# matinmoezzi/MyCobotGym

Measured on AMD Instinct MI355X. Metric: env-steps/sec (whole node), MyCobot Reach, N_envs=8192/GPU, higher is better.
Workload: dtype f64

## Files before the change

mycobotgym_amd/csrc/mcg_dynamics.hpp:

```cpp
#pragma once
#ifndef MCG_DUP
#define MCG_DUP 0
#endif

#include <type_traits>
#include <hip/hip_runtime.h>
#include "mcg.h"

namespace mcg {

typedef double real;

constexpr int NB = 12;
constexpr int AXK[NB] = {2, 0, 0, 0, 2, 0, 1, 1, 1, 1, 1, 1};
constexpr int AXS[NB] = {-1, -1, 1, -1, -1, -1, 1, -1, -1, 1, 1, 1};
constexpr int PAR[NB] = {-1, 0, 1, 2, 3, 4, 5, 6, 5, 8, 5, 5};
constexpr real MINVAL = 1e-15, MINIMP = 1e-4, MAXIMP = 0.9999;

#define MCG_DEV __device__ __forceinline__

enum { ST_LOAD = 0, ST_CTRL, ST_TRIG, ST_RNE, ST_ACT, ST_CRB, ST_ROWS, ST_G0, ST_NEWTON, ST_EULER, ST_COLLIDE, ST_CUBE,
       ST_COUPLED, ST_CUBE_FIN, ST_POST, ST_N_BUILD, ST_N_FACTOR, ST_N_SOLVE, ST_N_CHECK, ST_E_RHS, ST_R_AX5, ST_R_CONNECT, ST_R_LIMITS, ST_C_MASK, ST_C_ASSEMBLE, ST_C_SCHUR, ST_C_SOLVE, ST_C_CHECK, ST_C_LS, ST_W2_WAIT1, ST_W2_COLLIDE, ST_W2_CUBE, ST_W2_WAIT2, ST_W1_WAIT, ST_A_ENTRY, ST_A_G, ST_A_TWIST, ST_A_LOOP, ST_A_MAP, ST_A_STORE,
       ST_CO_SETUP, ST_CO_ROWS, ST_CO_H0, ST_CO_RESID, ST_CO_ASM, ST_CO_FACTOR, ST_CO_SOLVE, ST_CO_CHECK, ST_CO_LS, ST_CO_OUT, ST_CO_IDLE,
       ST_X_S1C, ST_X_NUMBERS, ST_X_S2, ST_S_S1B, ST_S_MESH, ST_S_S1C, ST_S_NUMBERS,
       ST_M_S3, ST_H_S1, ST_H_CRB, ST_H_S2, ST_H_FACTOR, ST_H_S3, ST_Q_S1, ST_Q_BIAS, ST_Q_S2, ST_Q_COLS, ST_Q_S3, ST_COUNT,
       CN_SUBSTEP = 0, CN_NEWTON_IT, CN_LINESEARCH, CN_CUBE_IT, CN_CUBE_LS, CN_COUPLED, CN_COUPLED_IT, CN_COUPLED_LS, CN_CONTACTS, CN_COOP_ROWS, CN_COOP_LSEVAL, CN_COOP_LONG, CN_COOP_CAP, CN_COOP_12, CN_G_FAILED, CN_G_LIM, CN_G_STAT, CN_G_CUBE, CN_G_MISSING, CN_G_EXTRA, CN_G_EQ1, CN_G_EQ2, CN_G_EQ2N1, CN_MP_PAIRS, CN_MP_HITS, CN_MP_FACE, CN_MP_EXIT_B, CN_MP_EXIT_P, CN_MP_EXIT_E, CN_MP_KIND_E, CN_MP_KIND_P, CN_MP_CUBE, CN_COUNT };
#ifdef MCG_STAGE_CLOCKS
__device__ unsigned long long g_stage_clocks[ST_COUNT + CN_COUNT];
__device__ unsigned long long g_tick_last[4096 * 4];
__device__ unsigned long long g_wg_stat[4096 * 4];
#define MCG_TICK_SLOT_ (g_tick_last[(blockIdx.x & 4095) * 4 + (threadIdx.x >> 6)])
#define MCG_TICK_INIT() do { if ((threadIdx.x & 63) == 0) MCG_TICK_SLOT_ = __builtin_readcyclecounter(); } while (0)
#define MCG_TICK(k) do { if ((threadIdx.x & 63) == 0) { const unsigned long long t_ = __builtin_readcyclecounter(); atomicAdd(&g_stage_clocks[k], t_ - MCG_TICK_SLOT_); MCG_TICK_SLOT_ = t_; } } while (0)
#define MCG_TICK2_INIT() MCG_TICK_INIT()
#define MCG_TICK2(k) MCG_TICK(k)
#define MCG_TICK_FLUSH() do {} while (0)
#define MCG_COUNT(k) do { if (threadIdx.x == 0) atomicAdd(&g_stage_clocks[ST_COUNT + (k)], 1ull); } while (0)
#define MCG_COUNTW(k, v) do { if ((threadIdx.x & 63) == 0) atomicAdd(&g_stage_clocks[ST_COUNT + (k)], (unsigned long long)(v)); } while (0)
#define MCG_TICK_PIN(arr, n) do { for (int k_ = 0; k_ < (n); k_++) asm volatile("" : "+v"((arr)[k_])); } while (0)
#else
#define MCG_TICK_INIT() do {} while (0)
#define MCG_TICK(k) do {} while (0)
#define MCG_TICK2_INIT() do {} while (0)
#define MCG_TICK2(k) do {} while (0)
#define MCG_TICK_FLUSH() do {} while (0)
#define MCG_COUNT(k) do {} while (0)
#define MCG_COUNTW(k, v) do {} while (0)
#define MCG_TICK_PIN(arr, n) do {} while (0)
#endif
template <int... Is, class F>
MCG_DEV void static_for_impl(std::integer_sequence<int, Is...>, F&& f) { (f(std::integral_constant<int, Is>{}), ...); }
template <int N, class F>
MCG_DEV void static_for(F&& f) { static_for_impl(std::make_integer_sequence<int, N>{}, f); }

MCG_DEV void cross(const real* a, const real* b, real* r) {
  real x = a[1] * b[2] - a[2] * b[1], y = a[2] * b[0] - a[0] * b[2], z = a[0] * b[1] - a[1] * b[0];
  r[0] = x; r[1] = y; r[2] = z;
}
// ... 261 lines not shown
}
template <int N>
MCG_DEV void chol_solve(const real* L, real* x) {
  static_for<N>([&](auto I) {
    constexpr int i = I;
    real s = x[i];
    static_for<i>([&](auto Kk) { constexpr int k = Kk; s -= L[i * (i + 1) / 2 + k] * x[k]; });
    x[i] = s / L[i * (i + 1) / 2 + i];
  });
  static_for<N>([&](auto I) {
    constexpr int i = N - 1 - I;
    real s = x[i];
    static_for<N - 1 - i>([&](auto Kk) { constexpr int k = i + 1 + Kk; s -= L[k * (k + 1) / 2 + i] * x[k]; });
    x[i] = s / L[i * (i + 1) / 2 + i];
  });
}

struct Robot {
  real q[NB], qd[NB], ctrl[7], warm[NB];
};

constexpr int LDS_M = 0;
constexpr int LDS_HEQ = NB * (NB + 1) / 2;
constexpr int LDS_SLOTS = 2 * (NB * (NB + 1) / 2);
constexpr int LDS_FAC = LDS_SLOTS, LDS_FDINV = LDS_FAC + NB * (NB + 1) / 2, LDS_QB = LDS_FDINV + NB, LDS_QDB = LDS_QB + NB;
constexpr int LDS_FS = LDS_QDB + NB, LDS_WARM = LDS_FS + NB, LDS_QLAG = LDS_WARM + NB, LDS_IKT = LDS_QLAG + 6;
constexpr int LDS_RLIM = LDS_WARM, LDS_RA = LDS_WARM, LDS_RACT = LDS_IKT, LDS_RG0 = LDS_IKT + 8, LDS_SLOTS_SPLIT = LDS_RG0 + NB;
constexpr int RACT_DOF[8] = {0, 1, 2, 3, 4, 5, 6, 8};
static_assert(LDS_RA + NB == LDS_QLAG && LDS_RACT >= LDS_QLAG + 6 && LDS_RACT + 8 <= LDS_RG0,
              "the remote solve's hand-over must stay inside the warm-start and IK-increment slots (the lagged q between them is live)");
static_assert(LDS_SLOTS_SPLIT * 64 * sizeof(real) <= 160 * 1024, "the split Reach kernel's LDS exceeds the 160 KB of a gfx950 workgroup");
constexpr int LDS_SN = LDS_FAC, LDS_CS = LDS_SN + NB;
static_assert(LDS_SN >= LDS_FAC && LDS_CS + NB <= LDS_FDINV + NB && LDS_FDINV + NB == LDS_QB, "the sine / cosine exchange must lie inside the factor slots");
template <class A, class B> MCG_DEV std::common_type_t<A, B> sel(bool c, A a, B b) { return c ? a : b; }
template <class T> MCG_DEV T sel3(int idx, T a, T b, T c) { return idx == 0 ? a : (idx == 1 ? b : c); }

#ifdef MCG_GENERIC_LDS
typedef real* LdsPtr;
#else
typedef __attribute__((address_space(3))) real* LdsPtr;
#endif
template <int STRIDE>
struct LaneScratchT {
  LdsPtr base;
  MCG_DEV explicit LaneScratchT(real* shared_column) : base((LdsPtr)shared_column) {}
  MCG_DEV explicit LaneScratchT(LdsPtr column) : base(column) {}
  MCG_DEV real ld(int k) const { return base[k * STRIDE]; }
  MCG_DEV void st(int k, real v) const { base[k * STRIDE] = v; }
};
typedef LaneScratchT<64> LaneScratch;

struct NoCoupling { static constexpr bool enabled = false, publishes = false; };
struct NoSideWork { MCG_DEV void operator()(const real*, const real*) const {} };

struct NoWeld { static constexpr bool enabled = false; };
struct Weld { static constexpr bool enabled = true; real pos[3], quat[4]; };

MCG_DEV void mulquat(const real* a, const real* b, real* r);
MCG_DEV void normalize4(real* q);
MCG_DEV void quat_to_mat(const real* q, real* m) {
  const real q00 = q[0]*q[0], q01 = q[0]*q[1], q02 = q[0]*q[2], q03 = q[0]*q[3];
  const real q11 = q[1]*q[1], q12 = q[1]*q[2], q13 = q[1]*q[3], q22 = q[2]*q[2], q23 = q[2]*q[3], q33 = q[3]*q[3];
  m[0] = q00 + q11 - q22 - q33; m[4] = q00 - q11 + q22 - q33; m[8] = q00 - q11 - q22 + q33;
  m[1] = 2*(q12 - q03); m[2] = 2*(q13 + q02); m[3] = 2*(q12 + q03);
  m[5] = 2*(q23 - q01); m[6] = 2*(q13 - q02); m[7] = 2*(q23 + q01);
}
// ... 148 lines not shown
        add[3] = It[3] - (m * r[0] * r[1] + r[0] * h3[1] + h3[0] * r[1]);
        add[4] = It[4] - (m * r[0] * r[2] + r[0] * h3[2] + h3[0] * r[2]);
        add[5] = It[5] - (m * r[1] * r[2] + r[1] * h3[2] + h3[1] * r[2]);
        if constexpr (first_child) {
          cm[p] = m;
          for (int k = 0; k < 3; k++) cmc[p][k] = h3[k] + m * r[k];
          for (int k = 0; k < 6; k++) cI[p][k] = add[k];
        } else {
          cm[p] += m;
          for (int k = 0; k < 3; k++) cmc[p][k] += h3[k] + m * r[k];
          for (int k = 0; k < 6; k++) cI[p][k] += add[k];
        }
        pin(cm[p]); pin3(cmc[p]); pin6(cI[p]);
      }
      asm volatile("" ::: "memory");
      MCG_FENCE();
    });
}

template <class LS>
MCG_DEV void euler_accel(ModelPtr Pm, real h, const LS MS, const real* a, real* rhs) {
  real Mh[NB * (NB + 1) / 2], dinv[NB];
  static_for<NB>([&](auto I) { constexpr int i = I;
    static_for<i + 1>([&](auto Jj) { constexpr int j = Jj; if constexpr (PAT_M.nz[i][j]) Mh[tri(i, j)] = MS.ld(LDS_M + tri(i, j)); }); });
  static_for<NB>([&](auto I) { constexpr int i = I; real sacc = 0;
    static_for<NB>([&](auto Jj) { constexpr int j = Jj;
      if constexpr (PAT_M.nz[i > j ? i : j][i > j ? j : i]) sacc = fma(Mh[tri(i, j)], a[j], sacc); }); rhs[i] = sacc; });
  { ModelPtr Q = launder(Pm); static_for<NB>([&](auto I) { constexpr int i = I; Mh[tri(i, i)] = fma(h, Q->body[i].damping, Mh[tri(i, i)]); }); }
  ldl_factor<PAT_M>(Mh, dinv);
  ldl_solve<PAT_M>(Mh, dinv, rhs);
}

struct NoSplit { static constexpr bool enabled = false, rne_remote = false, factor_remote = false, early_heq = false, warm_lds = false, mesh_split = false, solve_remote = false,
                                       trig_once = false;
                 static constexpr int QB = 0, QDB = 0, FS = 0, WARM = 0, QLAG = 0; };
struct SplitMain { static constexpr bool enabled = true, rne_remote = true, factor_remote = true, early_heq = true, warm_lds = true, mesh_split = false, solve_remote = true,
                                         trig_once = true;
                   static constexpr int QB = LDS_QB, QDB = LDS_QDB, FS = LDS_FS, WARM = LDS_WARM, QLAG = LDS_QLAG; };
struct SplitMainLocal : SplitMain { static constexpr bool solve_remote = false; };
struct SplitMainOwnTrig : SplitMain { static constexpr bool trig_once = false; };

template <int FIRST, class LS, class QF>
MCG_DEV void trig_exchange(const LS MS, QF q_of, real* sn, real* cs) {
  {
    const TrigC T = load_trig();
    static_for<4>([&](auto I) { constexpr int i = FIRST + I; real s, c; sincos_cw(T, AXS[i] * q_of(std::integral_constant<int, i>{}), s, c); MS.st(LDS_SN + i, s); MS.st(LDS_CS + i, c); });
  }
  __syncthreads();
  static_for<NB>([&](auto I) { constexpr int i = I; sn[i] = MS.ld(LDS_SN + i); cs[i] = MS.ld(LDS_CS + i); });
}

template <class SPL, class LS>
MCG_DEV void build_H(const LS MS, real* H, const bool* act_, const real* Dl) {
  static_for<NB>([&](auto I) { constexpr int i = I;
    static_for<i + 1>([&](auto Jj) { constexpr int j = Jj;
      if constexpr (PAT_E.nz[i][j]) {
        H[tri(i, j)] = MS.ld(LDS_HEQ + tri(i, j));
        if constexpr (SPL::early_heq && PAT_M.nz[i][j]) H[tri(i, j)] += MS.ld(LDS_M + tri(i, j));
      } else if constexpr (PAT_H.nz[i][j]) H[tri(i, j)] = 0.0; }); });
  static_for<10>([&](auto I) { constexpr int j = I; H[tri(j, j)] += act_[j] ? Dl[j] : 0.0; });
}

template <class SPL, class LS>
MCG_DEV bool no_other_rows(ModelPtr Pm, const LS MS) {
  real jr[10][2];
  { ModelPtr Q = launder(Pm); static_for<10>([&](auto I) { constexpr int j = I; if constexpr (j != 6 && j != 8) { jr[j][0] = Q->jnt_range[j][0]; jr[j][1] = Q->jnt_range[j][1]; } }); }
  bool other = false;
  static_for<10>([&](auto I) { constexpr int j = I;
    if constexpr (j != 6 && j != 8) {
      const real q = MS.ld(SPL::QB + j);
      other = other || (q - jr[j][0] < 0) || (jr[j][1] - q < 0);
    } });
// ... 2 lines not shown

MCG_DEV void limit_pair(bool e0, bool e1, real D0, real D1, real s0, real s1, real rb0, real rb1, real W00, real W01, real W11,
                        real& f0, real& f1) {
  const real A00 = rcp_nr(D0) + W00, A11 = rcp_nr(D1) + W11;
  const real n0 = rb0 * rcp_nr(A00), n1 = rb1 * rcp_nr(A11);
  const real idet = rcp_nr(A00 * A11 - W01 * W01);
  const real b0 = (A11 * rb0 - W01 * rb1) * idet, b1 = (A00 * rb1 - W01 * rb0) * idet;
  const bool cN = (!e0 || rb0 >= 0) && (!e1 || rb1 >= 0);
  const bool cB = e0 && e1 && (b0 < 0) && (b1 < 0);
  const bool c0 = e0 && (n0 < 0) && (!e1 || rb1 - W01 * n0 >= 0);
  const bool c1 = e1 && (n1 < 0) && (rb0 - W01 * n1 >= 0);
  real nu0 = e1 ? b0 : n0, nu1 = e1 ? b1 : 0.0;
  nu0 = c1 ? 0.0 : nu0; nu1 = c1 ? n1 : nu1;
  nu0 = c0 ? n0 : nu0;  nu1 = c0 ? 0.0 : nu1;
  nu0 = cB ? b0 : nu0;  nu1 = cB ? b1 : nu1;
  nu0 = cN ? 0.0 : nu0; nu1 = cN ? 0.0 : nu1;
  f0 = s0 * nu0; f1 = s1 * nu1;
}

MCG_DEV void gear_rows_solve(real* x, const real* z6, const real* z8, real Dl6, real arefl6, real sgl6, real Dl8, real arefl8, real sgl8) {
  const bool v6 = sgl6 != 0, v8 = sgl8 != 0, both = v6 && v8;
  const real D0 = v6 ? Dl6 : (v8 ? Dl8 : 1.0), D1 = both ? Dl8 : 1.0;
  const real ar0 = v6 ? arefl6 : arefl8, ar1 = both ? arefl8 : 0.0;
  const real s0 = v6 ? sgl6 : sgl8, s1 = both ? sgl8 : 0.0;
  const real xa0 = v6 ? x[6] : (v8 ? x[8] : 0.0), xa1 = both ? x[8] : 0.0;
  real W00 = v6 ? z6[6] : (v8 ? z8[8] : 0.0), W01 = both ? z6[8] : 0.0;
  const real W11 = both ? z8[8] : 0.0;
  W01 *= s0 * s1;
  const real rb0 = s0 * xa0 - ar0, rb1 = s1 * xa1 - ar1;
  real f0, f1;
  limit_pair(v6 || v8, both, D0, D1, s0, s1, rb0, rb1, W00, W01, W11, f0, f1);
  const real g6 = v6 ? f0 : 0.0, g8 = v6 ? f1 : f0;
  static_for<NB>([&](auto I) { constexpr int i = I; x[i] = fma(-z8[i], g8, fma(-z6[i], g6, x[i])); });
}

MCG_DEV bool bad_value(real x) { return !(fabs(x) <= 1e10); }

template <class LS, class CPL = NoCoupling, class WLD = NoWeld, class SPL = NoSplit, bool COMMIT = true>
MCG_DEV bool robot_substep(ModelPtr Pm, Robot& S, real* qlag6, const LS MS, CPL* CP = nullptr, const WLD* WD = nullptr,
                           Robot* next = nullptr) {
  MCG_COUNT(CN_SUBSTEP);
  if constexpr (SPL::enabled) __syncthreads();
  const real h = launder(Pm)->timestep;
  real cs[NB], sn[NB];
  if constexpr (SPL::trig_once) trig_exchange<0>(MS, [&](auto I) { return S.q[I]; }, sn, cs);
  else {
    const TrigC T = load_trig();
    static_for<NB>([&](auto I) { constexpr int i = I; sincos_cw(T, AXS[i] * S.q[i], sn[i], cs[i]); });
  }
  if constexpr (!(SPL::warm_lds && !CPL::enabled)) static_for<6>([&](auto I) { constexpr int i = I; qlag6[i] = S.q[i]; });
  static_for<NB>([&](auto I) { constexpr int i = I; pin(sn[i]); pin(cs[i]); });
  MCG_FENCE();

  MCG_TICK(ST_TRIG);
  real fs[NB];
  if constexpr (SPL::rne_remote) { static_for<NB>([&](auto I) { constexpr int i = I; fs[i] = 0; }); }
  else rne_bias(Pm, cs, sn, S.qd, fs);
  MCG_TICK(ST_RNE);
  {
    ModelPtr Q = launder(Pm);
    static_for<6>([&](auto I) {
      constexpr int u = I;
      real c = fmin(fmax(S.ctrl[u], Q->act_ctrlrange[u][0]), Q->act_ctrlrange[u][1]);
      real f = Q->act_gain[u] * c + Q->act_bias[u][0] + Q->act_bias[u][1] * S.q[u] + Q->act_bias[u][2] * S.qd[u];
      fs[u] += fmin(fmax(f, Q->act_forcerange[u][0]), Q->act_forcerange[u][1]);
    });
// ... 166 lines not shown
  };
  real g0[NB];
  static_for<NB>([&](auto I) { constexpr int i = I; g0[i] = 0; });
  static_for<2>([&](auto Sd) {
    constexpr int sd = Sd;
    constexpr int idx[9] = {0, 1, 2, 3, 4, 5, 6 + 2 * sd, 7 + 2 * sd, 10 + sd};
    static_for<3>([&](auto Kk) {
      constexpr int k = Kk; constexpr int ncol = (k == 1) ? 6 : 9;
      static_for<ncol>([&](auto A_) { constexpr int a = A_;
        g0[idx[a]] = fma(Dc[sd] * Jc[sd][k][a], arefc[sd][k], g0[idx[a]]); });
    });
  });
  g0[6] += Dj * arefj; g0[8] -= Dj * arefj;
  if constexpr (WLD::enabled)
    static_for<6>([&](auto Rr) { constexpr int r = Rr; const real da = Dw[r / 3] * arefw[r];
      static_for<6>([&](auto I) { constexpr int j = I; g0[j] = fma(Jw[r][j], da, g0[j]); }); });
  if constexpr (SPL::solve_remote) static_for<NB>([&](auto I) { constexpr int i = I; MS.st(LDS_RG0 + i, g0[i]); });
  if constexpr (SPL::early_heq) assemble_heq(std::false_type{});
#if MCG_DUP == 3
  if constexpr (SPL::early_heq && SPL::mesh_split) { MCG_FENCE(); static_for<2>([&](auto Sd) { constexpr int sd = Sd; pin(Dc[sd]); }); assemble_heq(std::false_type{}); }
#endif
  bool remote = false;
  if constexpr (SPL::solve_remote) {
    static_assert(!CPL::enabled && !SPL::mesh_split && SPL::rne_remote && SPL::factor_remote && SPL::early_heq && SPL::warm_lds,
                  "the remote solve replaces the direct solve of the three-wave Reach kernel; a coupled solve would skip it");
    bool other = false;
    static_for<10>([&](auto I) { constexpr int j = I; if constexpr (j != 6 && j != 8) other = other || (sgl[j] != 0); });
    remote = !__any(other);
    if (remote) {
#ifdef MCG_STAGE_CLOCKS
      MCG_COUNT(CN_NEWTON_IT);
      if (__any(sgl[6] != 0 || sgl[8] != 0)) MCG_COUNT(CN_LINESEARCH);
#endif
      static_for<2>([&](auto Sd) { constexpr int j = 6 + 2 * Sd;
        MS.st(LDS_RLIM + 3 * Sd, Dl[j]); MS.st(LDS_RLIM + 3 * Sd + 1, arefl[j]); MS.st(LDS_RLIM + 3 * Sd + 2, sgl[j]); });
    }
  }
  bool ahead = false;
  if constexpr (SPL::enabled) {
    if constexpr (SPL::mesh_split) {
      __syncthreads();
      ahead = __any(MS.ld(SPL::MASK0) != 0.0 || MS.ld(SPL::MASK0 + 1) != 0.0 || MS.ld(SPL::MASK0 + 2) != 0.0);
      if (!ahead) { __syncthreads(); __syncthreads(); }
    } else __syncthreads();
    if constexpr (SPL::solve_remote) {
      if (!remote) {
        static_for<NB>([&](auto I) { constexpr int i = I; fs[i] = 0; g0[i] = MS.ld(LDS_RG0 + i); });
        static_for<8>([&](auto K) { constexpr int k = K; fs[RACT_DOF[k]] = MS.ld(LDS_RACT + k); });
        static_for<NB>([&](auto I) { constexpr int i = I; fs[i] += MS.ld(SPL::FS + i); });
      }
    } else if constexpr (SPL::rne_remote) static_for<NB>([&](auto I) { constexpr int i = I; fs[i] += MS.ld(SPL::FS + i); });
  }
  static_for<NB>([&](auto I) { constexpr int i = I; g0[i] += fs[i]; });
  if constexpr (CPL::publishes) CP->publish(g0, Dl, arefl, sgl, S.qd, S.warm, !ahead);
  if constexpr (!SPL::early_heq) assemble_heq(std::true_type{});
  auto build_H = [&](real* H, const bool* act_) { mcg::build_H<SPL>(MS, H, act_, Dl); };

  MCG_TICK_PIN(g0, NB);
  MCG_TICK(ST_G0);
  real a[NB];
  bool act[10];
  if constexpr (SPL::warm_lds && !CPL::enabled) {
    static_for<NB>([&](auto I) { constexpr int i = I; a[i] = 0; });
    static_for<10>([&](auto I) { constexpr int j = I; act[j] = false; });
  } else {
    static_for<NB>([&](auto I) { constexpr int i = I; a[i] = S.warm[i]; });
// ... 101 lines not shown
    static_for<10>([&](auto I) { constexpr int j = I;
      const real rj = sgl[j] * a[j] - arefl[j], dj = sgl[j] * p[j];
      const real al_ = (sgl[j] != 0 && dj != 0) ? -rj / dj : -1.0;
      bp[j] = al_ > 0 ? al_ : INFINITY; });
    bool ls_done = false;
    for (int step = 0; step <= 10; step++) {
      real nxt = INFINITY; int jn = -1;
      static_for<10>([&](auto I) { constexpr int j = I; const bool lt = bp[j] < nxt; nxt = lt ? bp[j] : nxt; jn = lt ? j : jn; });
      const bool root = !ls_done && (slope > 0) && (val + slope * (nxt - alpha) >= 0);
      alpha = root ? alpha - val / slope : alpha;
      ls_done = ls_done || root;
      const bool none = !ls_done && (jn < 0);
      alpha = none ? 1.0 : alpha;
      ls_done = ls_done || none;
      const bool adv = !ls_done;
      val = adv ? val + slope * (nxt - alpha) : val;
      alpha = adv ? nxt : alpha;
      static_for<10>([&](auto I) { constexpr int j = I;
        const bool hit = adv && (j == jn);
        const real rj = sgl[j] * a[j] - arefl[j];
        const real dsl = Dl[j] * p[j] * p[j];
        slope = hit ? (rj < 0 ? slope - dsl : slope + dsl) : slope;
        bp[j] = hit ? INFINITY : bp[j]; });
    }
    static_for<NB>([&](auto I) { constexpr int i = I; a[i] = conv ? a[i] : fma(alpha, p[i], a[i]); });
    static_for<10>([&](auto I) { constexpr int j = I;
      const bool now = (sgl[j] != 0) && (sgl[j] * a[j] - arefl[j] < 0);
      act[j] = conv ? act[j] : now; });
  }

  MCG_TICK_PIN(a, NB);
  MCG_TICK(ST_NEWTON);
  real rhs[NB];
  if constexpr (SPL::factor_remote) {
    real damp[NB];
    if constexpr (SPL::solve_remote) {
      if (remote) { ModelPtr Q = launder(Pm); static_for<NB>([&](auto I) { constexpr int i = I; damp[i] = Q->body[i].damping; }); }
    }
    __syncthreads();
    MCG_TICK(ST_M_S3);
    if constexpr (SPL::solve_remote) { if (remote) static_for<NB>([&](auto I) { constexpr int i = I; a[i] = MS.ld(LDS_RA + i); }); }
    real Lf[NB * (NB + 1) / 2], dinv[NB];
    static_for<NB>([&](auto I) { constexpr int i = I; dinv[i] = MS.ld(LDS_FDINV + i);
      static_for<i>([&](auto Jj) { constexpr int j = Jj; if constexpr (PAT_M.nz[i][j]) Lf[tri(i, j)] = MS.ld(LDS_FAC + tri(i, j)); }); });
    if constexpr (SPL::solve_remote) {
      if (!remote) { ModelPtr Q = launder(Pm); static_for<NB>([&](auto I) { constexpr int i = I; damp[i] = Q->body[i].damping; }); }
      static_for<NB>([&](auto I) { constexpr int i = I; rhs[i] = damp[i] * a[i]; });
    } else { ModelPtr Q = launder(Pm); static_for<NB>([&](auto I) { constexpr int i = I; rhs[i] = Q->body[i].damping * a[i]; }); }
    ldl_solve<PAT_M>(Lf, dinv, rhs);
    static_for<NB>([&](auto I) { constexpr int i = I; rhs[i] = fma(-h, rhs[i], a[i]); });
  } else {
  MCG_TICK(ST_E_RHS);
  euler_accel(Pm, h, MS, a, rhs);
  }
  real qn[NB], qdn[NB];
  bool bad = false;
  static_for<NB>([&](auto I) { constexpr int i = I;
    real q_old, qd_old;
    if constexpr (SPL::warm_lds && !CPL::enabled) { q_old = MS.ld(SPL::QB + i); qd_old = MS.ld(SPL::QDB + i); if constexpr (i < 6) MS.st(SPL::QLAG + i, q_old); }
    else { q_old = S.q[i]; qd_old = S.qd[i]; }
    qdn[i] = fma(h, rhs[i], qd_old); qn[i] = fma(h, qdn[i], q_old);
    if constexpr (COMMIT) bad = bad || bad_value(qn[i]) || bad_value(qdn[i]) || bad_value(a[i]); });
  if constexpr (COMMIT) {
    if (__any(bad)) {
      static_for<NB>([&](auto I) { constexpr int i = I; qn[i] = sel(bad, 0.0, qn[i]); qdn[i] = sel(bad, 0.0, qdn[i]); a[i] = sel(bad, 0.0, a[i]); });
      static_for<7>([&](auto I) { constexpr int k = I; S.ctrl[k] = sel(bad, 0.0, S.ctrl[k]); });
    }
  }
  static_for<NB>([&](auto I) { constexpr int i = I;
    const real qd_new = qdn[i], q_new = qn[i];
    if constexpr (COMMIT) { S.qd[i] = qd_new; S.q[i] = q_new; if constexpr (SPL::warm_lds && !CPL::enabled) MS.st(SPL::WARM + i, a[i]); else S.warm[i] = a[i]; }
    else { next->qd[i] = qd_new; next->q[i] = q_new; next->warm[i] = a[i]; }
    if constexpr (SPL::enabled && COMMIT) { MS.st(SPL::QB + i, q_new); MS.st(SPL::QDB + i, qd_new); } });
  MCG_TICK_PIN(S.q, NB); MCG_TICK_PIN(S.qd, NB);
  MCG_TICK(ST_EULER);
  if constexpr (SPL::enabled && SPL::mesh_split) { if (ahead) { __syncthreads(); __syncthreads(); } }
  return bad;
}

template <class SPL, int FIRST, class LS>
MCG_DEV void side_trig(const LS MS, real* sn, real* cs) {
  if constexpr (SPL::trig_once) trig_exchange<FIRST>(MS, [&](auto I) { return MS.ld(SPL::QB + I); }, sn, cs);
  else {
    const TrigC T = load_trig();
    static_for<NB>([&](auto I) { constexpr int i = I; sincos_cw(T, AXS[i] * MS.ld(SPL::QB + i), sn[i], cs[i]); });
  }
  static_for<NB>([&](auto I) { constexpr int i = I; pin(sn[i]); pin(cs[i]); });
  MCG_FENCE();
}

template <class SPL = SplitMain, class LS, class SIDE = NoSideWork>
MCG_DEV void helper_substep(ModelPtr Pm, const LS MS, const SIDE& side = SIDE{}) {
  __syncthreads();
  MCG_TICK(ST_H_S1);
  real cs[NB], sn[NB];
  side_trig<SPL, 4>(MS, sn, cs);
  crb_to_lds(Pm, cs, sn, MS);
  static_assert(!SPL::mesh_split, "the four-wave PickAndPlace kernel drives its side waves itself: helper_pre / rne_pre");
  (void)side;
  MCG_TICK(ST_H_CRB);
  __syncthreads();
  MCG_TICK(ST_H_S2);
  if constexpr (SPL::factor_remote) {
    const real h = launder(Pm)->timestep;
    real Mh[NB * (NB + 1) / 2], dinv[NB];
    static_for<NB>([&](auto I) { constexpr int i = I;
      static_for<i + 1>([&](auto Jj) { constexpr int j = Jj; if constexpr (PAT_M.nz[i][j]) Mh[tri(i, j)] = MS.ld(LDS_M + tri(i, j)); }); });
    { ModelPtr Q = launder(Pm); static_for<NB>([&](auto I) { constexpr int i = I; Mh[tri(i, i)] = fma(h, Q->body[i].damping, Mh[tri(i, i)]); }); }
    ldl_factor<PAT_M>(Mh, dinv);
    static_for<NB>([&](auto I) { constexpr int i = I; MS.st(LDS_FDINV + i, dinv[i]);
      static_for<i>([&](auto Jj) { constexpr int j = Jj; if constexpr (PAT_M.nz[i][j]) MS.st(LDS_FAC + tri(i, j), Mh[tri(i, j)]); }); });
    MCG_TICK(ST_H_FACTOR);
    __syncthreads();
    MCG_TICK(ST_H_S3);
  }
}

template <class SPL = SplitMain, class LS, class SIDE = NoSideWork>
MCG_DEV void rne_substep(ModelPtr Pm, const LS MS, const SIDE& side = SIDE{}) {
  __syncthreads();
  MCG_TICK(ST_Q_S1);
  real cs[NB], sn[NB], qd[NB], fs[NB];
  side_trig<SPL, 8>(MS, sn, cs);
  static_for<NB>([&](auto I) { constexpr int i = I; qd[i] = MS.ld(SPL::QDB + i); });
  rne_bias(Pm, cs, sn, qd, fs);
  static_for<NB>([&](auto I) { constexpr int i = I; MS.st(SPL::FS + i, fs[i]); });
  bool remote = false;
  if constexpr (SPL::solve_remote) {
    remote = no_other_rows<SPL>(Pm, MS);
    static_for<NB>([&](auto I) { constexpr int i = I; pin(fs[i]); });
    MCG_FENCE();
  }
  static_assert(!SPL::mesh_split, "the four-wave PickAndPlace kernel drives its side waves itself: helper_pre / rne_pre");
  (void)side;
  MCG_TICK(ST_Q_BIAS);
  __syncthreads();
  MCG_TICK(ST_Q_S2);
  if constexpr (SPL::solve_remote) {
    if (remote) {
      real L[NB * (NB + 1) / 2], dinv[NB], x[NB];
      const bool none[10] = {false, false, false, false, false, false, false, false, false, false};
      const real zero[10] = {0, 0, 0, 0, 0, 0, 0, 0, 0, 0};
      build_H<SPL>(MS, L, none, zero);
      static_for<NB>([&](auto I) { constexpr int i = I; x[i] = 0.0; });
      static_for<8>([&](auto K) { constexpr int k = K; x[RACT_DOF[k]] = MS.ld(LDS_RACT + k); });
      static_for<NB>([&](auto I) { constexpr int i = I; x[i] = MS.ld(LDS_RG0 + i) + (x[i] + fs[i]); });
      ldl_factor<PAT_H>(L, dinv);
      ldl_solve<PAT_H>(L, dinv, x);
      const real Dl6 = MS.ld(LDS_RLIM), arefl6 = MS.ld(LDS_RLIM + 1), sgl6 = MS.ld(LDS_RLIM + 2);
      const real Dl8 = MS.ld(LDS_RLIM + 3), arefl8 = MS.ld(LDS_RLIM + 4), sgl8 = MS.ld(LDS_RLIM + 5);
      if (__any(sgl6 != 0 || sgl8 != 0)) {
        real z6[NB], z8[NB];
        ldl_solve_unit<PAT_H, 6>(L, dinv, z6);
        ldl_solve_unit<PAT_H, 8>(L, dinv, z8);
        static_for<NB>([&](auto I) { constexpr int i = I; pin(z6[i]); pin(z8[i]); });
        gear_rows_solve(x, z6, z8, Dl6, arefl6, sgl6, Dl8, arefl8, sgl8);
      }
      static_for<NB>([&](auto I) { constexpr int i = I; MS.st(LDS_RA + i, x[i]); });
      MCG_TICK(ST_Q_COLS);
    }
  }
  if constexpr (SPL::factor_remote) __syncthreads();
  MCG_TICK(ST_Q_S3);
}

template <class SPL, class LS, class SIDE>
MCG_DEV void helper_pre(ModelPtr Pm, const LS MS, const SIDE& side) {
  __syncthreads();
  MCG_TICK(ST_C_CHECK);
  real cs[NB], sn[NB];
  {
    const TrigC T = load_trig();
    static_for<NB>([&](auto I) { constexpr int i = I; sincos_cw(T, AXS[i] * MS.ld(SPL::QB + i), sn[i], cs[i]); });
  }
  static_for<NB>([&](auto I) { constexpr int i = I; pin(sn[i]); pin(cs[i]); });
  MCG_FENCE();
  crb_to_lds(Pm, cs, sn, MS);
  MCG_TICK(ST_C_MASK);
  side(sn, cs);
  MCG_TICK(ST_C_ASSEMBLE);
}
template <class SPL, class LS, class SIDE>
MCG_DEV void rne_pre(ModelPtr Pm, const LS MS, const SIDE& side) {
  __syncthreads();
  MCG_TICK(ST_C_CHECK);
  real cs[NB], sn[NB], qd[NB], fs[NB];
  {
    const TrigC T = load_trig();
    static_for<NB>([&](auto I) { constexpr int i = I; sincos_cw(T, AXS[i] * MS.ld(SPL::QB + i), sn[i], cs[i]); qd[i] = MS.ld(SPL::QDB + i); });
// ... 115 lines not shown
```

mycobotgym_amd/csrc/mcg_hip.hip:

```cpp
#include <hip/hip_runtime.h>
#include <cstdlib>
#include <cstddef>
#include <cmath>
#include <cstdarg>
#include <cstdio>
#include <cstring>
#include <new>
#include <vector>

#include "mcg.h"
#include "mcg_engine.hpp"
#include "mcg_dynamics.hpp"
#include "mcg_cube.hpp"
#include "mcg_coop.hpp"
#include "model_gen.h"
#include "polytopes_gen.h"

using namespace mcg;

namespace {

struct Env {
  Robot R;
  real qlag6[6], goal[3], epret;
// ... 75 lines not shown
  for (int k = 0; k < 3; k++) E.goal[k] = V.goal(k, i);
  E.epret = V.epret(i); E.elapsed = V.elapsed(i); E.episode = V.episode(i); E.eplen = V.eplen(i);
}
MCG_DEV void load_env(const View& V, int i, Env& E) { load_robot(V, i, E); load_episode(V, i, E); }
MCG_DEV void store_env(const View& V, int i, const Env& E) {
  for (int k = 0; k < NB; k++) { V.qpos(k, i) = E.R.q[k]; V.qvel(k, i) = E.R.qd[k]; V.warm(k, i) = E.R.warm[k]; }
  for (int k = 0; k < 7; k++) V.ctrl(k, i) = E.R.ctrl[k];
  for (int k = 0; k < 6; k++) V.qlag(k, i) = E.qlag6[k];
  for (int k = 0; k < 3; k++) V.goal(k, i) = E.goal[k];
  V.epret(i) = E.epret; V.elapsed(i) = E.elapsed; V.episode(i) = E.episode; V.eplen(i) = E.eplen;
}

MCG_DEV void write_obs(const mcg_step_out& O, int i, int D, const real* obs, const real* ag, const real* goal) {
  if (O.obs) for (int k = 0; k < D; k++) O.obs[(size_t)i * D + k] = obs[k];
  if (O.achieved_goal) for (int k = 0; k < 3; k++) O.achieved_goal[(size_t)i * 3 + k] = ag[k];
  if (O.desired_goal) for (int k = 0; k < 3; k++) O.desired_goal[(size_t)i * 3 + k] = goal[k];
}

MCG_DEV void mocap_target(const Cfg& C, ModelPtr P, const real* qlag6, const float* act, Weld& W) {
  TcpPose X; tcp_forward(P, qlag6, X, false);
  for (int k = 0; k < 3; k++) W.pos[k] = X.pos[k] + (real)(act[k] * 0.1f);
  const real fq[4] = {0.5, -0.5, -0.5, 0.5};
  for (int k = 0; k < 4; k++) {
    const real qt = C.fetch ? fq[k] : (real)act[3 + k];
    const real dq = qt - X.quat[k];
    W.quat[k] = X.quat[k] + dq;
  }
  normalize4(W.quat);
}

#ifndef MCG_SOLVE_REMOTE_CTRLS
#define MCG_SOLVE_REMOTE_CTRLS (1 << MCG_CTRL_JOINT)
#endif

template <int CONTROLLER, bool SPLIT>
__global__ __launch_bounds__(SPLIT ? 192 : 64) void step_reach_kernel(Cfg C, View V, const mcg_model* __restrict__ Pg,
                                                                      const float* __restrict__ actions, mcg_step_out O) {
  typedef std::conditional_t<SPLIT, std::conditional_t<(MCG_SOLVE_REMOTE_CTRLS >> CONTROLLER) & 1, SplitMain, SplitMainLocal>, NoSplit> Split;
  __shared__ real lds[SPLIT ? LDS_SLOTS_SPLIT : LDS_SLOTS][64];
  const int lane = threadIdx.x & 63;
  const LaneScratch MS(&lds[0][lane]);
  const ModelPtr P = as_model_ptr(Pg);
  const int i = blockIdx.x * 64 + lane;
  if (i >= C.n) return;
  if constexpr (SPLIT) {
    if (threadIdx.x >= 64) {
      MCG_TICK_INIT();
      if constexpr (CONTROLLER == MCG_CTRL_IK) {
        if (threadIdx.x < 128) {
          for (int c = 0; c < C.control_steps; c++) { __syncthreads(); __syncthreads(); for (int s = 0; s < C.frame_skip; s++) helper_substep<Split>(P, MS); }
        } else {
          float act[8];
          _Pragma("unroll") for (int k = 0; k < 8; k++) {
            const float x = (k < C.act_dim) ? actions[(size_t)i * C.act_dim + (k < C.act_dim ? k : 0)] : 0.f;
            act[k] = fminf(fmaxf(x, -1.f), 1.f);
          }
          real tpos[3], tquat[4];
          for (int c = 0; c < C.control_steps; c++) {
            __syncthreads();
            real ql[6]; EefPose X;
            for (int k = 0; k < 6; k++) ql[k] = MS.ld(LDS_QLAG + k);
            eef_forward(P, ql, X, true);
            if (c == 0) {
              for (int k = 0; k < 3; k++) tpos[k] = X.pos[k] + (real)(act[k] * 0.2f);
              if (C.fetch) { tquat[0] = 0; tquat[1] = -0.707; tquat[2] = 0; tquat[3] = 0.707; }
              else {
                real e[3], qr[4], cur[4];
                for (int k = 0; k < 3; k++) e[k] = (real)(act[3 + k] * 0.5f);
                euler2quat(e, qr); mat2quat(X.mat, cur); mulquat(qr, cur, tquat);
              }
            }
// ... 213 lines not shown
  E.dr[0] = sel(doit, drs[0], E.dr[0]); E.dr[1] = sel(doit, drs[1], E.dr[1]);
  E.elapsed = sel(doit, 0, E.elapsed); E.epret = sel(doit, 0.0, E.epret); E.eplen = sel(doit, 0, E.eplen);
  E.episode += sel(doit, 1, 0);
}

MCG_DEV void observe_pnp(const Cfg& C, ModelPtr P, const EnvP& E, real* obs, real* ag) {
  EefPose X;
  eef_forward(P, E.qlag6, X, true);
  real gv[3];
  for (int k = 0; k < 3; k++) { real v = 0; for (int j = 0; j < 6; j++) v += X.jacp[k][j] * E.R.qd[j]; gv[k] = v * C.dt; }
  real Rl[9], eul[3];
  quat_to_mat(E.qlag7 + 3, Rl); mat2euler(Rl, eul);
  for (int k = 0; k < 3; k++) {
    obs[k] = X.pos[k]; obs[3 + k] = E.qlag7[k]; obs[6 + k] = E.qlag7[k] - X.pos[k];
    obs[11 + k] = eul[k];
    obs[14 + k] = E.Cb.vel[k] * C.dt - gv[k];
    obs[17 + k] = (Rl[3*k]*E.Cb.vel[3] + Rl[3*k+1]*E.Cb.vel[4] + Rl[3*k+2]*E.Cb.vel[5]) * C.dt;
    obs[20 + k] = gv[k];
    ag[k] = E.qlag7[k];
  }
  obs[9] = E.R.q[6]; obs[10] = E.R.q[8];
  obs[23] = E.R.qd[6] * C.dt; obs[24] = E.R.qd[8] * C.dt;
}

MCG_DEV void hide_object(real* obs, real* ag) {
  const real o[10] = {obs[0], obs[1], obs[2], obs[9], obs[10], obs[20], obs[21], obs[22], obs[23], obs[24]};
  for (int k = 0; k < 10; k++) obs[k] = o[k];
  for (int k = 0; k < 3; k++) ag[k] = o[k];
}

constexpr int XCH_FS = PNP_SLOTS;
constexpr int PNP_SLOTS_DUAL = PNP_SLOTS_LDS;
static_assert(PNP_SLOTS_DUAL * PNP_LANES * 8 <= 160 * 1024, "LDS of a CU");
struct SplitPnp { static constexpr bool enabled = true, rne_remote = true, factor_remote = false, early_heq = true, warm_lds = false, mesh_split = true, solve_remote = false, trig_once = false;
                  static constexpr int QB = XCH_Q, QDB = XCH_QD, FS = XCH_FS, WARM = 0, QLAG = 0, MASK0 = MP_MASK; };

MCG_DEV bool flag_coupled(real f) { return (((int)f) & 2) != 0; }
MCG_DEV bool flag_cube_bad(real f) { return (((int)f) & 8) != 0; }

struct PubHook {
  static constexpr bool enabled = false, publishes = true;
  const PnpScratch S;
  MCG_DEV void publish(const real* g0, const real* Dl, const real* arefl, const real* sgl, const real* qd, const real* warm, bool flags_known) const {
    const bool flag = !flags_known || flag_coupled(S.ld(XCH_FLAG));
    if (__any(flag)) {
      if (flag) {
        static_for<NB>([&](auto I) { constexpr int k = I; S.st(PUB_G0 + k, g0[k]); S.st(PUB_WARM + k, warm[k]); });
        static_for<10>([&](auto I) { constexpr int j = I; S.st(PUB_SD + j, sgl[j] * Dl[j]); S.st(pub_aref(j), arefl[j]); });
      }
    }
  }
};

MCG_DEV void cube_to_lds(const PnpScratch MS, const Cube& Cb) {
  for (int k = 0; k < 3; k++) MS.st(XCH_CB + k, Cb.pos[k]);
  for (int k = 0; k < 4; k++) MS.st(XCH_CB + 3 + k, Cb.quat[k]);
  for (int k = 0; k < 6; k++) { MS.st(XCH_CB + 7 + k, Cb.vel[k]); MS.st(XCH_CB + 13 + k, Cb.warm[k]); }
}
MCG_DEV void cube_from_lds(const PnpScratch MS, Cube& Cb) {
  for (int k = 0; k < 3; k++) Cb.pos[k] = MS.ld(XCH_CB + k);
  for (int k = 0; k < 4; k++) Cb.quat[k] = MS.ld(XCH_CB + 3 + k);
  for (int k = 0; k < 6; k++) { Cb.vel[k] = MS.ld(XCH_CB + 7 + k); Cb.warm[k] = MS.ld(XCH_CB + 13 + k); }
}
MCG_DEV unsigned flagged_lanes(const PnpScratch MS, int nvalid) {
  return (unsigned)__ballot(flag_coupled(MS.ld(XCH_FLAG))) & (nvalid >= 32 ? 0xFFFFFFFFu : ((1u << nvalid) - 1u));
}

// ... 741 lines not shown
```

Before: 43.24 million.

## Move gear-row unit columns to helper wave and mass factor to main wave

Adds a SplitMainCols policy, on by default for the joint controller. In it the helper wave factors the unconstrained H and publishes its unit-solve columns z6/z8 through LDS. The main wave factors M+hD itself and applies the gear-row correction locally, instead of the remote solver doing the factor and the limit correction. This rebalances work between the cooperating waves so the remote solve's critical path gets shorter. In exchange the main wave does more register-heavy work and there are more LDS slot aliasing constraints.

```diff
diff --git a/mycobotgym_amd/csrc/mcg_dynamics.hpp b/mycobotgym_amd/csrc/mcg_dynamics.hpp
--- a/mycobotgym_amd/csrc/mcg_dynamics.hpp
+++ b/mycobotgym_amd/csrc/mcg_dynamics.hpp
@@ -23,7 +23,7 @@
        ST_COUPLED, ST_CUBE_FIN, ST_POST, ST_N_BUILD, ST_N_FACTOR, ST_N_SOLVE, ST_N_CHECK, ST_E_RHS, ST_R_AX5, ST_R_CONNECT, ST_R_LIMITS, ST_C_MASK, ST_C_ASSEMBLE, ST_C_SCHUR, ST_C_SOLVE, ST_C_CHECK, ST_C_LS, ST_W2_WAIT1, ST_W2_COLLIDE, ST_W2_CUBE, ST_W2_WAIT2, ST_W1_WAIT, ST_A_ENTRY, ST_A_G, ST_A_TWIST, ST_A_LOOP, ST_A_MAP, ST_A_STORE,
        ST_CO_SETUP, ST_CO_ROWS, ST_CO_H0, ST_CO_RESID, ST_CO_ASM, ST_CO_FACTOR, ST_CO_SOLVE, ST_CO_CHECK, ST_CO_LS, ST_CO_OUT, ST_CO_IDLE,
        ST_X_S1C, ST_X_NUMBERS, ST_X_S2, ST_S_S1B, ST_S_MESH, ST_S_S1C, ST_S_NUMBERS,
-       ST_M_S3, ST_H_S1, ST_H_CRB, ST_H_S2, ST_H_FACTOR, ST_H_S3, ST_Q_S1, ST_Q_BIAS, ST_Q_S2, ST_Q_COLS, ST_Q_S3, ST_COUNT,
+       ST_M_S3, ST_H_S1, ST_H_CRB, ST_H_S2, ST_H_FACTOR, ST_H_S3, ST_Q_S1, ST_Q_BIAS, ST_Q_S2, ST_Q_COLS, ST_Q_S3, ST_M_FACTOR, ST_H_COLS, ST_M_GEAR, ST_COUNT,
        CN_SUBSTEP = 0, CN_NEWTON_IT, CN_LINESEARCH, CN_CUBE_IT, CN_CUBE_LS, CN_COUPLED, CN_COUPLED_IT, CN_COUPLED_LS, CN_CONTACTS, CN_COOP_ROWS, CN_COOP_LSEVAL, CN_COOP_LONG, CN_COOP_CAP, CN_COOP_12, CN_G_FAILED, CN_G_LIM, CN_G_STAT, CN_G_CUBE, CN_G_MISSING, CN_G_EXTRA, CN_G_EQ1, CN_G_EQ2, CN_G_EQ2N1, CN_MP_PAIRS, CN_MP_HITS, CN_MP_FACE, CN_MP_EXIT_B, CN_MP_EXIT_P, CN_MP_EXIT_E, CN_MP_KIND_E, CN_MP_KIND_P, CN_MP_CUBE, CN_COUNT };
 #ifdef MCG_STAGE_CLOCKS
 __device__ unsigned long long g_stage_clocks[ST_COUNT + CN_COUNT];
@@ -351,6 +351,9 @@
 static_assert(LDS_SLOTS_SPLIT * 64 * sizeof(real) <= 160 * 1024, "the split Reach kernel's LDS exceeds the 160 KB of a gfx950 workgroup");
 constexpr int LDS_SN = LDS_FAC, LDS_CS = LDS_SN + NB;
 static_assert(LDS_SN >= LDS_FAC && LDS_CS + NB <= LDS_FDINV + NB && LDS_FDINV + NB == LDS_QB, "the sine / cosine exchange must lie inside the factor slots");
+constexpr int LDS_Z6 = LDS_CS + NB, LDS_Z8 = LDS_Z6 + NB;
+static_assert(LDS_Z6 == LDS_FAC + 24 && LDS_Z6 >= LDS_SN + NB && LDS_Z6 >= LDS_CS + NB && LDS_Z8 == LDS_Z6 + NB && LDS_Z8 + NB <= LDS_QB,
+              "the gear rows' columns must lie inside the factor slots, clear of the sine / cosine exchange and of the published q");
 template <class A, class B> MCG_DEV std::common_type_t<A, B> sel(bool c, A a, B b) { return c ? a : b; }
 template <class T> MCG_DEV T sel3(int idx, T a, T b, T c) { return idx == 0 ? a : (idx == 1 ? b : c); }
 
@@ -565,12 +568,13 @@
 }
 
 struct NoSplit { static constexpr bool enabled = false, rne_remote = false, factor_remote = false, early_heq = false, warm_lds = false, mesh_split = false, solve_remote = false,
-                                       trig_once = false;
+                                       trig_once = false, helper_cols = false;
                  static constexpr int QB = 0, QDB = 0, FS = 0, WARM = 0, QLAG = 0; };
 struct SplitMain { static constexpr bool enabled = true, rne_remote = true, factor_remote = true, early_heq = true, warm_lds = true, mesh_split = false, solve_remote = true,
-                                         trig_once = true;
+                                         trig_once = true, helper_cols = false;
                    static constexpr int QB = LDS_QB, QDB = LDS_QDB, FS = LDS_FS, WARM = LDS_WARM, QLAG = LDS_QLAG; };
 struct SplitMainLocal : SplitMain { static constexpr bool solve_remote = false; };
+struct SplitMainCols : SplitMain { static constexpr bool helper_cols = true; };
 struct SplitMainOwnTrig : SplitMain { static constexpr bool trig_once = false; };
 
 template <int FIRST, class LS, class QF>
@@ -639,6 +643,14 @@
   limit_pair(v6 || v8, both, D0, D1, s0, s1, rb0, rb1, W00, W01, W11, f0, f1);
   const real g6 = v6 ? f0 : 0.0, g8 = v6 ? f1 : f0;
   static_for<NB>([&](auto I) { constexpr int i = I; x[i] = fma(-z8[i], g8, fma(-z6[i], g6, x[i])); });
+}
+
+template <class LS>
+MCG_DEV void factor_m_hb(ModelPtr Pm, const LS MS, real h, real* Mh, real* dinv, real* damp) {
+  static_for<NB>([&](auto I) { constexpr int i = I;
+    static_for<i + 1>([&](auto Jj) { constexpr int j = Jj; if constexpr (PAT_M.nz[i][j]) Mh[tri(i, j)] = MS.ld(LDS_M + tri(i, j)); }); });
+  { ModelPtr Q = launder(Pm); static_for<NB>([&](auto I) { constexpr int i = I; damp[i] = Q->body[i].damping; Mh[tri(i, i)] = fma(h, damp[i], Mh[tri(i, i)]); }); }
+  ldl_factor<PAT_M>(Mh, dinv);
 }
 
 MCG_DEV bool bad_value(real x) { return !(fabs(x) <= 1e10); }
@@ -871,6 +883,7 @@
       MCG_COUNT(CN_NEWTON_IT);
       if (__any(sgl[6] != 0 || sgl[8] != 0)) MCG_COUNT(CN_LINESEARCH);
 #endif
+      if constexpr (!SPL::helper_cols)
       static_for<2>([&](auto Sd) { constexpr int j = 6 + 2 * Sd;
         MS.st(LDS_RLIM + 3 * Sd, Dl[j]); MS.st(LDS_RLIM + 3 * Sd + 1, arefl[j]); MS.st(LDS_RLIM + 3 * Sd + 2, sgl[j]); });
     }
@@ -1038,7 +1051,32 @@
   MCG_TICK_PIN(a, NB);
   MCG_TICK(ST_NEWTON);
   real rhs[NB];
-  if constexpr (SPL::factor_remote) {
+  real q_pre[NB], qd_pre[NB];
+  if constexpr (SPL::helper_cols) {
+    static_assert(SPL::solve_remote && SPL::factor_remote, "helper_cols moves pieces of the remote solve and of the remote factor");
+    real Lf[NB * (NB + 1) / 2], dinv[NB], damp[NB];
+    factor_m_hb(Pm, MS, h, Lf, dinv, damp);
+    static_for<NB>([&](auto I) { constexpr int i = I; q_pre[i] = MS.ld(SPL::QB + i); qd_pre[i] = MS.ld(SPL::QDB + i); if constexpr (i < 6) MS.st(SPL::QLAG + i, q_pre[i]); });
+    static_for<NB>([&](auto I) { constexpr int i = I; pin(dinv[i]);
+      static_for<i>([&](auto Jj) { constexpr int j = Jj; if constexpr (PAT_M.nz[i][j]) pin(Lf[tri(i, j)]); }); });
+    MCG_FENCE();
+    MCG_TICK(ST_M_FACTOR);
+    __syncthreads();
+    MCG_TICK(ST_M_S3);
+    if (remote) {
+      static_for<NB>([&](auto I) { constexpr int i = I; a[i] = MS.ld(LDS_RA + i); });
+      if (__any(sgl[6] != 0 || sgl[8] != 0)) {
+        real z6[NB], z8[NB];
+        static_for<NB>([&](auto I) { constexpr int i = I; z6[i] = MS.ld(LDS_Z6 + i); z8[i] = MS.ld(LDS_Z8 + i); });
+        gear_rows_solve(a, z6, z8, Dl[6], arefl[6], sgl[6], Dl[8], arefl[8], sgl[8]);
+      }
+      MCG_TICK_PIN(a, NB);
+      MCG_TICK(ST_M_GEAR);
+    }
+    static_for<NB>([&](auto I) { constexpr int i = I; rhs[i] = damp[i] * a[i]; });
+    ldl_solve<PAT_M>(Lf, dinv, rhs);
+    static_for<NB>([&](auto I) { constexpr int i = I; rhs[i] = fma(-h, rhs[i], a[i]); });
+  } else if constexpr (SPL::factor_remote) {
     real damp[NB];
     if constexpr (SPL::solve_remote) {
       if (remote) { ModelPtr Q = launder(Pm); static_for<NB>([&](auto I) { constexpr int i = I; damp[i] = Q->body[i].damping; }); }
@@ -1063,7 +1101,8 @@
   bool bad = false;
   static_for<NB>([&](auto I) { constexpr int i = I;
     real q_old, qd_old;
-    if constexpr (SPL::warm_lds && !CPL::enabled) { q_old = MS.ld(SPL::QB + i); qd_old = MS.ld(SPL::QDB + i); if constexpr (i < 6) MS.st(SPL::QLAG + i, q_old); }
+    if constexpr (SPL::helper_cols) { q_old = q_pre[i]; qd_old = qd_pre[i]; }
+    else if constexpr (SPL::warm_lds && !CPL::enabled) { q_old = MS.ld(SPL::QB + i); qd_old = MS.ld(SPL::QDB + i); if constexpr (i < 6) MS.st(SPL::QLAG + i, q_old); }
     else { q_old = S.q[i]; qd_old = S.qd[i]; }
     qdn[i] = fma(h, rhs[i], qd_old); qn[i] = fma(h, qdn[i], q_old);
     if constexpr (COMMIT) bad = bad || bad_value(qn[i]) || bad_value(qdn[i]) || bad_value(a[i]); });
@@ -1107,13 +1146,22 @@
   MCG_TICK(ST_H_CRB);
   __syncthreads();
   MCG_TICK(ST_H_S2);
-  if constexpr (SPL::factor_remote) {
+  if constexpr (SPL::helper_cols) {
+    real L[NB * (NB + 1) / 2], dinv[NB], z6[NB], z8[NB];
+    const bool none[10] = {false, false, false, false, false, false, false, false, false, false};
+    const real zero[10] = {0, 0, 0, 0, 0, 0, 0, 0, 0, 0};
+    build_H<SPL>(MS, L, none, zero);
+    ldl_factor<PAT_H>(L, dinv);
+    ldl_solve_unit<PAT_H, 6>(L, dinv, z6);
+    ldl_solve_unit<PAT_H, 8>(L, dinv, z8);
+    static_for<NB>([&](auto I) { constexpr int i = I; MS.st(LDS_Z6 + i, z6[i]); MS.st(LDS_Z8 + i, z8[i]); });
+    MCG_TICK(ST_H_COLS);
+    __syncthreads();
+    MCG_TICK(ST_H_S3);
+  } else if constexpr (SPL::factor_remote) {
     const real h = launder(Pm)->timestep;
-    real Mh[NB * (NB + 1) / 2], dinv[NB];
-    static_for<NB>([&](auto I) { constexpr int i = I;
-      static_for<i + 1>([&](auto Jj) { constexpr int j = Jj; if constexpr (PAT_M.nz[i][j]) Mh[tri(i, j)] = MS.ld(LDS_M + tri(i, j)); }); });
-    { ModelPtr Q = launder(Pm); static_for<NB>([&](auto I) { constexpr int i = I; Mh[tri(i, i)] = fma(h, Q->body[i].damping, Mh[tri(i, i)]); }); }
-    ldl_factor<PAT_M>(Mh, dinv);
+    real Mh[NB * (NB + 1) / 2], dinv[NB], damp[NB];
+    factor_m_hb(Pm, MS, h, Mh, dinv, damp);
     static_for<NB>([&](auto I) { constexpr int i = I; MS.st(LDS_FDINV + i, dinv[i]);
       static_for<i>([&](auto Jj) { constexpr int j = Jj; if constexpr (PAT_M.nz[i][j]) MS.st(LDS_FAC + tri(i, j), Mh[tri(i, j)]); }); });
     MCG_TICK(ST_H_FACTOR);
@@ -1153,6 +1201,7 @@
       static_for<NB>([&](auto I) { constexpr int i = I; x[i] = MS.ld(LDS_RG0 + i) + (x[i] + fs[i]); });
       ldl_factor<PAT_H>(L, dinv);
       ldl_solve<PAT_H>(L, dinv, x);
+      if constexpr (!SPL::helper_cols) {
       const real Dl6 = MS.ld(LDS_RLIM), arefl6 = MS.ld(LDS_RLIM + 1), sgl6 = MS.ld(LDS_RLIM + 2);
       const real Dl8 = MS.ld(LDS_RLIM + 3), arefl8 = MS.ld(LDS_RLIM + 4), sgl8 = MS.ld(LDS_RLIM + 5);
       if (__any(sgl6 != 0 || sgl8 != 0)) {
@@ -1161,6 +1210,7 @@
         ldl_solve_unit<PAT_H, 8>(L, dinv, z8);
         static_for<NB>([&](auto I) { constexpr int i = I; pin(z6[i]); pin(z8[i]); });
         gear_rows_solve(x, z6, z8, Dl6, arefl6, sgl6, Dl8, arefl8, sgl8);
+      }
       }
       static_for<NB>([&](auto I) { constexpr int i = I; MS.st(LDS_RA + i, x[i]); });
       MCG_TICK(ST_Q_COLS);
diff --git a/mycobotgym_amd/csrc/mcg_hip.hip b/mycobotgym_amd/csrc/mcg_hip.hip
--- a/mycobotgym_amd/csrc/mcg_hip.hip
+++ b/mycobotgym_amd/csrc/mcg_hip.hip
@@ -131,11 +131,15 @@
 #ifndef MCG_SOLVE_REMOTE_CTRLS
 #define MCG_SOLVE_REMOTE_CTRLS (1 << MCG_CTRL_JOINT)
 #endif
+#ifndef MCG_HELPER_COLS_CTRLS
+#define MCG_HELPER_COLS_CTRLS (1 << MCG_CTRL_JOINT)
+#endif
 
 template <int CONTROLLER, bool SPLIT>
 __global__ __launch_bounds__(SPLIT ? 192 : 64) void step_reach_kernel(Cfg C, View V, const mcg_model* __restrict__ Pg,
                                                                       const float* __restrict__ actions, mcg_step_out O) {
-  typedef std::conditional_t<SPLIT, std::conditional_t<(MCG_SOLVE_REMOTE_CTRLS >> CONTROLLER) & 1, SplitMain, SplitMainLocal>, NoSplit> Split;
+  typedef std::conditional_t<SPLIT, std::conditional_t<(MCG_SOLVE_REMOTE_CTRLS >> CONTROLLER) & 1,
+                                                      std::conditional_t<(MCG_HELPER_COLS_CTRLS >> CONTROLLER) & 1, SplitMainCols, SplitMain>, SplitMainLocal>, NoSplit> Split;
   __shared__ real lds[SPLIT ? LDS_SLOTS_SPLIT : LDS_SLOTS][64];
   const int lane = threadIdx.x & 63;
   const LaneScratch MS(&lds[0][lane]);
@@ -415,7 +419,7 @@
 constexpr int XCH_FS = PNP_SLOTS;
 constexpr int PNP_SLOTS_DUAL = PNP_SLOTS_LDS;
 static_assert(PNP_SLOTS_DUAL * PNP_LANES * 8 <= 160 * 1024, "LDS of a CU");
-struct SplitPnp { static constexpr bool enabled = true, rne_remote = true, factor_remote = false, early_heq = true, warm_lds = false, mesh_split = true, solve_remote = false, trig_once = false;
+struct SplitPnp { static constexpr bool enabled = true, rne_remote = true, factor_remote = false, early_heq = true, warm_lds = false, mesh_split = true, solve_remote = false, trig_once = false, helper_cols = false;
                   static constexpr int QB = XCH_Q, QDB = XCH_QD, FS = XCH_FS, WARM = 0, QLAG = 0, MASK0 = MP_MASK; };
 
 MCG_DEV bool flag_coupled(real f) { return (((int)f) & 2) != 0; }
```

After: 44.40 million, median of 6. 1.03x the previous value.
